# arnaucube/go-snark-study

Hardware: AMD Instinct MI355X
Metric: Groth16 constraints/sec (prove) at 2^20 R1CS (higher is better)
Workload: dtype u32 (9x29-bit Montgomery limbs of the 254-bit BN128 fields)

## Files before the change

go-snark-study_amd/csrc/msm.hip:

```cpp
#include "msm.h"
#include "hostcopy.h"

#include <algorithm>
#include <cmath>
#include <cstdlib>
#include <future>
#include <type_traits>

#include "msm_kernels.h"

namespace gs {

static_assert(sizeof(G1Xyzz) == PointIO<FqTag>::kXyzzWords * 4, "G1 XYZZ must be raw limbs");
static_assert(sizeof(G2Xyzz) == PointIO<Fq2Tag>::kXyzzWords * 4, "G2 XYZZ must be raw limbs");

int choose_window_bits(uint32_t n, int forced) {
  if (forced >= 8 && forced <= kMaxWindowBits) return forced;
  static const double per_bucket = dev_knob_f("GS_WINDOW_COST_BUCKET", 6.0, 0.0, 64.0);
  static const int auto_max = (int)dev_knob("GS_AUTO_MAX_C", 17, 8, kMaxWindowBits);
  int best = 8;
  double best_cost = 1e300;
  for (int c = 8; c <= std::min(kMaxWindowBits, std::max(8, auto_max)); ++c) {
    const int W = 254 / c + 1;
    const double cost = (double)n * W + per_bucket * (double)(1u << (c - 1));
    if (cost < best_cost) { best_cost = cost; best = c; }
  }
  return best;
}

int choose_window_bits_free(uint32_t n, int forced) {
  if (forced) return std::min(kMaxFreeWindowBits, std::max(kMinFreeWindowBits, forced));
  static const double per_bucket = dev_knob_f("GS_WINDOW_COST_BUCKET_FREE", 3.0, 0.0, 64.0);
  int best = kMinFreeWindowBits;
  double best_cost = 1e300;
  for (int c = kMinFreeWindowBits; c <= kMaxFreeWindowBits; ++c) {
    const int W = 254 / c + 1;
    const double cost = (double)W * ((double)n + per_bucket * (double)(1u << (c - 1)));
    if (cost < best_cost) { best_cost = cost; best = c; }
  }
  return best;
}

static void exclusive_scan(Ctx& c, PlanBuffers& pb, const uint32_t* in, uint32_t* out, uint32_t n) {
  const uint32_t ntiles = (n + kScanTile - 1) / kScanTile;
  pb.tiles.ensure((size_t)ntiles * 4);
  pb.total.ensure(4);
  hipLaunchKernelGGL(k_scan_tiles, dim3(ntiles), dim3(kScanBlock), 0, c.stream, in, out, pb.tiles.as<uint32_t>(), n);
  hipLaunchKernelGGL(k_scan_tile_sums, dim3(1), dim3(1024), 0, c.stream, pb.tiles.as<uint32_t>(), ntiles, pb.total.as<uint32_t>());
  hipLaunchKernelGGL(k_scan_add, dim3(ntiles), dim3(kScanBlock), 0, c.stream, out, pb.tiles.as<uint32_t>(), n);
}

struct MsmState {
  PlanBuffers plan_slots[3 * Ctx::kSlots];
  DevBuf upload_scratch;
  DevBuf upload_flag;
  bool lds_attr_set = false;
};
static MsmState& msm_state(Ctx& c) { return c.state<MsmState>(c.msm_state); }

static uint32_t choose_chunk(uint64_t entries, uint32_t nbuckets, const std::vector<LaunchShape>& users) {
  static const int forced = (int)dev_knob("GS_CHUNK", 0, 4, 1024, 4);
  if (forced >= 4 && forced % 4 == 0) return (uint32_t)forced;
  static const int forced_h = (int)dev_knob("GS_CHUNK_H", 0, 4, 1024, 4);
  if (forced_h && users.size() == 1 && users[0].njobs == 1 && !users[0].g2) return (uint32_t)forced_h;
  uint32_t chunk = entries >= (1ull << 27) ? 64u : entries >= (1ull << 23) ? 32u : 16u;
  while (chunk < 1024u && entries / std::max<uint32_t>(nbuckets, 1u) > 32ull * chunk) chunk *= 2;
  return chunk;
}

static uint32_t part_min_ranges() {
  static const uint32_t v = (uint32_t)dev_knob("GS_PART_MIN_R", 4, 2, 64);
  return v;
}
bool plan_partitions_first(int cbits) {
  if (cbits < 1) return false;
  return std::max<uint32_t>(1u, (1u << (cbits - 1)) >> kRangeLog) >= part_min_ranges();
}

uint32_t finite_mask_dev(Ctx& c, const uint32_t* g1_pts, const uint32_t* g2_pts, uint32_t n, uint32_t* mask_dev) {
  const size_t words = ((size_t)n + 31) / 32;
  GS_HIP(hipMemsetAsync(mask_dev, 0, std::max<size_t>(words, 1) * 4, c.stream));
  DevBuf cnt(4);
  GS_HIP(hipMemsetAsync(cnt.p, 0, 4, c.stream));
  if (n) hipLaunchKernelGGL(k_finite_mask, grid1(n), dim3(256), 0, c.stream, g1_pts, (uint32_t)PointIO<FqTag>::kAffineWords, g2_pts,
                            (uint32_t)PointIO<Fq2Tag>::kAffineWords, n, mask_dev, cnt.as<uint32_t>());
  GS_HIP(hipGetLastError());
  uint32_t host = 0;
  GS_HIP(hipMemcpyAsync(&host, cnt.p, 4, hipMemcpyDeviceToHost, c.stream));
  GS_HIP(hipStreamSynchronize(c.stream));
  return host;
}

void build_plan(Ctx& c, int slot, const uint32_t* scalars_dev, uint32_t n, MsmPlan& plan, const std::vector<LaunchShape>& users, int cbits,
                bool table_free, const uint32_t* term_index, uint32_t index_bias) {
  MsmState& ms = msm_state(c);
  PlanBuffers& pb = ms.plan_slots[slot % (3 * Ctx::kSlots)];
  plan.n = n;
  plan.table_free = table_free;
  plan.c = cbits ? cbits : (table_free ? choose_window_bits_free(n, c.window_bits) : choose_window_bits(n, c.window_bits));
  if (table_free && (plan.c < kMinFreeWindowBits || plan.c > kMaxFreeWindowBits))
    throw HipError{hipErrorInvalidValue, "table-free plan outside 9..16 window bits", __LINE__};
  plan.W = 254 / plan.c + 1;
  plan.B = 1u << (plan.c - 1);
  plan.nbuckets = table_free ? (uint32_t)plan.W * plan.B : plan.B;
  plan.chunk = choose_chunk((uint64_t)n * plan.W, plan.nbuckets, users);
  plan.maxchunks = (uint32_t)(((size_t)n * plan.W + plan.chunk - 1) / plan.chunk) + 1;
  const size_t ncount = (size_t)plan.nbuckets + 1;
  PlanParams pp{};
  pp.n = n; pp.c = plan.c; pp.W = plan.W; pp.B = plan.B;
  pp.R = std::max<uint32_t>(1u, plan.B >> kRangeLog);
  pp.tf = table_free ? 1u : 0u;
  {
    const uint32_t want = std::max<uint32_t>(1u, 256u / (plan.W * pp.R));
    const uint32_t by_size = std::max<uint32_t>(1u, (n + 16383u) / 16384u);
    const uint32_t by_mem = std::max<uint32_t>(1u, (uint32_t)((64ull << 20) / ((uint64_t)plan.B * plan.W * 4)));
    pp.S = std::max<uint32_t>(1u, std::min(std::min<uint32_t>(16u, std::max<uint32_t>(want, 1u)), std::min(by_size, by_mem)));
    if (pp.R == 1 && !table_free) pp.S = std::max<uint32_t>(1u, std::min<uint32_t>(16u, by_size));
  }
  pp.slice = (n + pp.S - 1) / pp.S;
  pp.stride = (n + 63u) & ~63u;
  const bool wide = plan_partitions_first(plan.c);
  if (wide && term_index) throw HipError{hipErrorInvalidValue, "plans over a term list cannot be sorted partition-first (plan_partitions_first)", __LINE__};
  const uint32_t nparts = (uint32_t)plan.W * pp.R;
  if (wide && nparts > kMaxParts) throw HipError{hipErrorInvalidValue, "too many (window, range) partitions", __LINE__};
  if (!wide) pb.digits.ensure((size_t)std::max<uint32_t>(pp.stride, 64u) * plan.W * sizeof(digit_t));
  else {
    pb.recs.ensure(std::max<size_t>((size_t)n * plan.W, 1) * 8);
    pb.parts.ensure((size_t)(3 * kMaxParts + 4) * 4);
  }
  pb.hist.ensure((size_t)plan.B * plan.W * pp.S * 4);
  pb.totals.ensure(ncount * 4);
  pb.offsets.ensure(ncount * 4);
  pb.entries.ensure(((size_t)plan.maxchunks + 1) * plan.chunk * 4);
  pb.chunk_bucket.ensure((size_t)plan.maxchunks * 4);
  pb.heavy_list.ensure((size_t)plan.nbuckets * 4);
  pb.counters.ensure(16);
  const size_t lds = (size_t)std::min<uint32_t>(plan.B, kRangeBuckets) * 4;
  static const int sort_block = (int)dev_knob("GS_SORT_BLOCK", kSortBlock, 64, kSortBlock, 64);
  if (!ms.lds_attr_set) {
    GS_HIP(hipFuncSetAttribute(reinterpret_cast<const void*>(k_hist), hipFuncAttributeMaxDynamicSharedMemorySize, 128 * 1024));
    GS_HIP(hipFuncSetAttribute(reinterpret_cast<const void*>(k_scatter), hipFuncAttributeMaxDynamicSharedMemorySize, 128 * 1024));
    GS_HIP(hipFuncSetAttribute(reinterpret_cast<const void*>(k_hist_part), hipFuncAttributeMaxDynamicSharedMemorySize, 128 * 1024));
    GS_HIP(hipFuncSetAttribute(reinterpret_cast<const void*>(k_scatter_part), hipFuncAttributeMaxDynamicSharedMemorySize, 128 * 1024));
    ms.lds_attr_set = true;
  }
  GS_HIP(hipMemsetAsync(pb.totals.as<uint32_t>() + plan.nbuckets, 0, 4, c.stream));
  GS_HIP(hipMemsetAsync(pb.counters.p, 0, 16, c.stream));
  uint32_t* part_count = pb.parts.as<uint32_t>();
  uint32_t* part_base = part_count ? part_count + kMaxParts : nullptr;
  uint32_t* part_cursor = part_count ? part_base + kMaxParts + 4 : nullptr;
  if (n > 0 && wide) {
    GS_HIP(hipMemsetAsync(part_count, 0, (size_t)nparts * 4, c.stream));
    hipLaunchKernelGGL(k_part_count, grid1(n, kPartBlock), dim3(kPartBlock), 0, c.stream, scalars_dev, pp, part_count);
    hipLaunchKernelGGL(k_part_scan, dim3(1), dim3(64), 0, c.stream, part_count, nparts, part_base, part_cursor);
    hipLaunchKernelGGL(k_part_scatter, grid1(n, kPartBlock * kPartPerThread), dim3(kPartBlock), 0, c.stream, scalars_dev, pp, part_base, part_cursor,
                       pb.recs.as<uint2>());
    hipLaunchKernelGGL(k_hist_part, dim3(8 * pp.S * ((nparts + 7) / 8)), dim3(sort_block), lds, c.stream, pb.recs.as<uint2>(), part_base, pp, pb.hist.as<uint32_t>());
    hipLaunchKernelGGL(k_colscan, grid1(plan.B), dim3(256), 0, c.stream, pb.hist.as<uint32_t>(), pp, pb.totals.as<uint32_t>());
  } else if (n > 0) {
    hipLaunchKernelGGL(k_digits, grid1(n), dim3(256), 0, c.stream, scalars_dev, pp, pb.digits.as<digit_t>(), term_index, index_bias);
    hipLaunchKernelGGL(k_hist, dim3(plan.W, pp.S, pp.R), dim3(sort_block), lds, c.stream, pb.digits.as<digit_t>(), pp, pb.hist.as<uint32_t>());
    if (table_free) hipLaunchKernelGGL(k_colscan_windows, grid1(plan.nbuckets), dim3(256), 0, c.stream, pb.hist.as<uint32_t>(), pp, pb.totals.as<uint32_t>());
    else hipLaunchKernelGGL(k_colscan, grid1(plan.B), dim3(256), 0, c.stream, pb.hist.as<uint32_t>(), pp, pb.totals.as<uint32_t>());
  } else {
    GS_HIP(hipMemsetAsync(pb.totals.p, 0, ncount * 4, c.stream));
  }
  exclusive_scan(c, pb, pb.totals.as<uint32_t>(), pb.offsets.as<uint32_t>(), (uint32_t)ncount);
  if (n > 0) {
    if (wide) hipLaunchKernelGGL(k_scatter_part, dim3(8 * pp.S * ((nparts + 7) / 8)), dim3(sort_block), lds, c.stream, pb.recs.as<uint2>(), part_base, pp,
                                 pb.hist.as<uint32_t>(), pb.offsets.as<uint32_t>(), pb.entries.as<uint32_t>());
    else hipLaunchKernelGGL(k_scatter, dim3(plan.W, pp.S, pp.R), dim3(sort_block), lds, c.stream, pb.digits.as<digit_t>(), pp, pb.hist.as<uint32_t>(),
                            pb.offsets.as<uint32_t>(), pb.entries.as<uint32_t>(), term_index, index_bias);
    hipLaunchKernelGGL(k_chunk_map, grid1(plan.nbuckets), dim3(256), 0, c.stream, pb.offsets.as<uint32_t>(), plan.nbuckets, plan.chunk,
                       pb.chunk_bucket.as<uint32_t>(), pb.heavy_list.as<uint32_t>(), pb.counters.as<uint32_t>());
  }
  GS_HIP(hipGetLastError());
  plan.offsets = pb.offsets.as<uint32_t>();
  plan.entries = pb.entries.as<uint32_t>();
  plan.chunk_bucket = pb.chunk_bucket.as<uint32_t>();
  plan.heavy_list = pb.heavy_list.as<uint32_t>();
  plan.heavy_count = pb.counters.as<uint32_t>();
}

template <class T>
static void msm_enqueue(Ctx& c, const MsmPlan& plan, const std::vector<MsmBase>& bases, int ws_base, int slot, MsmPending& p,
                        hipStream_t tail_stream) {
  const int njobs = (int)bases.size();
  p = MsmPending{};
  p.njobs = njobs; p.slot = slot; p.n = plan.n; p.g2 = PointIO<T>::kAffineWords == 32;
  p.c = plan.c; p.W = plan.W;
  if (njobs == 0 || plan.n == 0) { p.njobs = plan.n == 0 ? -njobs : 0; return; }
  if (njobs > kMaxJobs) throw HipError{hipErrorInvalidValue, "too many MSM jobs", __LINE__};
  constexpr size_t pw = PointIO<T>::kXyzzWords;
  constexpr size_t aw = PointIO<T>::kAffineWords;
  static const uint32_t fold_env = (uint32_t)dev_knob("GS_FOLD_MAX", 0, 1, 256);
  const uint32_t fold_max = fold_env ? fold_env : (plan.n >= (1u << 19) ? 32u : 16u);
  static const uint32_t l_min = (uint32_t)dev_knob("GS_REDUCE_L", 4, 1, 32, 1, true);
  int L = (int)std::max<uint32_t>(1u, std::min<uint32_t>(l_min, plan.B / kReduceBlock));
  while (L < 32 && plan.B / ((uint32_t)kReduceBlock * (uint32_t)L) > fold_max) L *= 2;
  uint32_t nblk = (plan.B + kReduceBlock * L - 1) / (kReduceBlock * L);
  if (plan.table_free) {
    L = (int)std::max<uint32_t>(1u, std::min<uint32_t>(16u, plan.B / kReduceBlock));
    p.nblk_window = plan.B / ((uint32_t)kReduceBlock * (uint32_t)L);
    nblk = p.nblk_window * (uint32_t)plan.W;
    p.table_free = true;
  }
  p.L = L; p.nblk = nblk;
  p.folded = !plan.table_free && nblk > fold_max;
  if (p.folded && nblk > (uint32_t)kReduceBlock) throw HipError{hipErrorInvalidValue, "too many reduce workgroups for one fold", __LINE__};
  const size_t pair_bytes = (size_t)njobs * nblk * 2 * pw * 4, final_bytes = (size_t)njobs * pw * 4, stats_bytes = 16;
  const size_t out_bytes = (p.folded ? final_bytes : pair_bytes + final_bytes) + stats_bytes;
  if (out_bytes > Ctx::kPinnedBytes) throw HipError{hipErrorInvalidValue, "MSM result staging too small", __LINE__};
  p.stats_off = out_bytes - stats_bytes;
  AccJobs jobs{};
  DevBuf& outb = c.ws_out[ws_base % Ctx::kWsSets];
  outb.ensure(pair_bytes + final_bytes + stats_bytes);
  uint32_t* finals = outb.as<uint32_t>() + pair_bytes / 4;
  uint32_t* stats = finals + final_bytes / 4;
  for (int j = 0; j < njobs; ++j) {
    const BaseTable* t = bases[j].table;
    const uint32_t* points = nullptr;
    uint32_t row_stride = 0;
    if (plan.table_free) {
      if (!bases[j].points || bases[j].off + plan.n > bases[j].npoints)
        throw HipError{hipErrorInvalidValue, "MSM base array does not cover the plan", __LINE__};
      points = bases[j].points + bases[j].off * aw;
    } else {
      if (!t || t->c != plan.c || !t->rows.p || bases[j].off + plan.n > t->n)
        throw HipError{hipErrorInvalidValue, "MSM base table does not match the plan", __LINE__};
      points = t->rows.as<uint32_t>() + bases[j].off * aw;
      row_stride = (uint32_t)t->n;
    }
    DevBuf& bk = c.ws_buckets[(ws_base + j) % Ctx::kWsSets];
    DevBuf& mg = c.ws_chunks[(ws_base + j) % Ctx::kWsSets];
    DevBuf& pt = c.ws_partials[(ws_base + j) % Ctx::kWsSets];
    bk.ensure((size_t)plan.nbuckets * pw * 4);
    mg.ensure((size_t)plan.nbuckets * pw * 4);
    pt.ensure((size_t)plan.maxchunks * 2 * pw * 4);
    jobs.j[j] = AccJob{points, row_stride, bk.as<uint32_t>(), pt.as<uint32_t>(),
                       pt.as<uint32_t>() + (size_t)plan.maxchunks * pw, mg.as<uint32_t>(),
                       outb.as<uint32_t>() + (size_t)j * nblk * 2 * pw, finals + (size_t)j * pw};
  }
  p.tacc = std::make_shared<PhaseTimer>(c.stream);
  p.tker = std::make_shared<PhaseTimer>(c.stream);
  hipLaunchKernelGGL(k_bucket_accumulate<T>, dim3((plan.maxchunks + kAccBlock - 1) / kAccBlock, njobs), dim3(kAccBlock), 0, c.stream,
                     jobs, plan.offsets, plan.entries, plan.chunk_bucket, plan.nbuckets, plan.chunk);
  p.tker->stop();
  p.tacc->stop();
  hipStream_t ts = tail_stream ? tail_stream : c.stream;
  if (ts != c.stream) {
    hipEvent_t ev;
    GS_HIP(hipEventCreateWithFlags(&ev, hipEventDisableTiming));
    GS_HIP(hipEventRecord(ev, c.stream));
    GS_HIP(hipStreamWaitEvent(ts, ev, 0));
    GS_HIP(hipEventDestroy(ev));
  }
  p.tred = std::make_shared<PhaseTimer>(ts);
  static const long alone_below_log2 = dev_knob("GS_TAIL_ALONE_LOG2", 19, 0, 32);
  const bool alone = plan.n < (1ull << alone_below_log2);
  auto launch_tails = [&](auto alone_tag) {
    constexpr bool kAlone = decltype(alone_tag)::value;
    hipLaunchKernelGGL((k_heavy_combine<T, kAlone>), dim3(64, njobs), dim3(kHeavyBlock), 0, ts,
                       jobs, plan.offsets, plan.heavy_list, plan.heavy_count, plan.chunk);
    hipLaunchKernelGGL((k_heavy_finish<T, kAlone>), dim3(16, njobs), dim3(kHeavyBlock), 0, ts,
                       jobs, plan.offsets, plan.heavy_list, plan.heavy_count, plan.chunk);
    hipLaunchKernelGGL((k_bucket_combine<T, kAlone>), dim3((plan.nbuckets + 255) / 256, njobs), dim3(256), 0, ts, jobs, plan.offsets, plan.nbuckets,
                       plan.chunk, plan.heavy_count, stats);
    hipLaunchKernelGGL((k_block_reduce<T, kAlone>), dim3(nblk, njobs), dim3(kReduceBlock), 0, ts, jobs, plan.nbuckets, L);
    if (p.folded) {
      int log2_span = 0;
      while ((1u << log2_span) < (uint32_t)kReduceBlock * (uint32_t)L) ++log2_span;
      hipLaunchKernelGGL((k_pair_reduce<T, kAlone>), dim3(1, njobs), dim3(kReduceBlock), 0, ts, jobs, nblk, log2_span);
    }
  };
  if (alone) launch_tails(std::true_type{}); else launch_tails(std::false_type{});
  GS_HIP(hipGetLastError());
  GS_HIP(hipMemcpyAsync(c.pinned[slot], p.folded ? (const void*)finals : outb.p, out_bytes, hipMemcpyDeviceToHost, ts));
  p.pinned_slot = c.pinned[slot];
  p.tred->stop();
}

template <class T>
static Xyzz<T> sum_pairs(const Xyzz<T>* pr, uint32_t nblk, int L) {
  Xyzz<T> run = xyzz_inf<T>(), tot = xyzz_inf<T>(), sumA = xyzz_inf<T>();
  for (uint32_t blk = nblk; blk-- > 0;) {
    xyzz_add(sumA, pr[2 * blk]);
    if (blk >= 1) { xyzz_add(run, pr[2 * blk + 1]); xyzz_add(tot, run); }
  }
  for (uint32_t s2 = (uint32_t)kReduceBlock * (uint32_t)L; s2 > 1; s2 >>= 1) xyzz_dbl(tot);
  xyzz_add(sumA, tot);
  return sumA;
}

void msm_book_timing(Ctx& c, const MsmPending& p) {
  if (p.njobs <= 0) return;
  std::lock_guard<std::mutex> lk(c.timing_mu);
  c.timing.accumulate_ms += p.tacc->ms();
  const uint64_t terms = (uint64_t)p.n * p.njobs;
  c.timing.window_bits = (uint32_t)p.c;
  c.timing.reduce_ms += p.tred->ms();
  const uint32_t* st = p.pinned_slot ? reinterpret_cast<const uint32_t*>(static_cast<const char*>(p.pinned_slot) + p.stats_off) : nullptr;
  const uint64_t adds = st ? (uint64_t)st[0] * p.njobs : terms * p.W;
  if (!p.g2) { c.timing.acc_g1_ms += p.tker->ms(); c.timing.acc_g1_launches += 1; c.timing.acc_g1_terms += terms; c.timing.acc_g1_adds += adds; }
  else { c.timing.acc_g2_ms += p.tker->ms(); c.timing.acc_g2_launches += 1; c.timing.acc_g2_terms += terms; c.timing.acc_g2_adds += adds; }
  c.timing.plan_digits += terms * p.W;
  c.timing.plan_entries += adds;
  if (st) c.timing.heavy_buckets += st[1];
}

template <class T>
static Xyzz<T> sum_pairs_windows(const Xyzz<T>* pr, const MsmPending& p) {
  Xyzz<T> acc = xyzz_inf<T>();
  for (int w = p.W; w-- > 0;) {
    for (int k = 0; k < p.c; ++k) xyzz_dbl(acc);
    xyzz_add(acc, sum_pairs<T>(pr + (size_t)w * p.nblk_window * 2, p.nblk_window, p.L));
  }
  return acc;
}

template <class T>
static void msm_finish(Ctx& c, const MsmPending& p, std::vector<Xyzz<T>>& out) {
  if (p.njobs <= 0) { out.assign(-p.njobs, xyzz_inf<T>()); return; }
  out.assign(p.njobs, xyzz_inf<T>());
  const Xyzz<T>* pairs = static_cast<const Xyzz<T>*>(c.pinned[p.slot]);
  if (p.folded) {
// ... 187 lines not shown
```

go-snark-study_amd/csrc/msm_kernels.h:

```cpp
#pragma once
#include <hip/hip_runtime.h>
#include <stdint.h>

#include "ec.h"
#include "point_io.h"
#include "zkey_convert.h"

namespace gs {

struct PlanParams {
  uint32_t n;
  int c;
  int W;
  uint32_t B;
  uint32_t S;
  uint32_t slice;
  uint32_t stride;
  uint32_t R;
  uint32_t tf;
};
constexpr uint32_t kRangeLog = 15;
constexpr uint32_t kRangeBuckets = 1u << kRangeLog;

GS_HD int32_t next_digit(const uint32_t (&k)[8], const PlanParams& pp, int w, uint32_t& carry) {
  uint32_t raw = scalar_bits(k, w * pp.c, pp.c) + carry;
  if (raw > pp.B) { carry = 1; return (int32_t)raw - (int32_t)(2u * pp.B); }
  carry = 0;
  return (int32_t)raw;
}

using digit_t = uint32_t;
__global__ void __launch_bounds__(256) k_digits(const uint32_t* __restrict__ scalars, PlanParams pp, digit_t* __restrict__ digits,
                                                 const uint32_t* __restrict__ term_index, uint32_t index_bias) {
  wave_priority<GS_PRIO_PLAN>();
  const uint32_t i = blockIdx.x * blockDim.x + threadIdx.x;
  if (i >= pp.n) return;
  const uint32_t src = term_index ? term_index[i] - index_bias : i;
  uint32_t k[8];
  const uint4* s4 = reinterpret_cast<const uint4*>(scalars + (size_t)src * 8);
  uint4 lo = s4[0], hi = s4[1];
  k[0] = lo.x; k[1] = lo.y; k[2] = lo.z; k[3] = lo.w; k[4] = hi.x; k[5] = hi.y; k[6] = hi.z; k[7] = hi.w;
  scalar_canon(k);
  uint32_t carry = 0;
  for (int w = 0; w < pp.W; ++w) {
    const int32_t d = next_digit(k, pp, w, carry);
    digits[(size_t)w * pp.stride + i] = (digit_t)(d + (int32_t)pp.B - 1);
  }
}

__global__ void __launch_bounds__(256) k_finite_mask(const uint32_t* __restrict__ a, uint32_t wa, const uint32_t* __restrict__ b, uint32_t wb, uint32_t n,
                                                      uint32_t* __restrict__ mask, uint32_t* __restrict__ count) {
  const uint32_t i = blockIdx.x * blockDim.x + threadIdx.x;
  bool finite = false;
  if (i < n) {
    uint32_t acc = 0;
    if (a) for (uint32_t k = 0; k < wa; ++k) acc |= a[(size_t)i * wa + k];
    if (b) for (uint32_t k = 0; k < wb; ++k) acc |= b[(size_t)i * wb + k];
    finite = acc != 0;
  }
  if (finite) { atomicOr(&mask[i >> 5], 1u << (i & 31u)); atomicAdd(count, 1u); }
}

constexpr int kSortBlock = 1024;

__global__ void __launch_bounds__(kSortBlock) k_hist(const digit_t* __restrict__ digits, PlanParams pp, uint32_t* __restrict__ hist) {
  wave_priority<GS_PRIO_PLAN>();
  extern __shared__ uint32_t sh[];
  const uint32_t w = blockIdx.x, s = blockIdx.y, r = blockIdx.z;
  const uint32_t nb = min(pp.B, kRangeBuckets), base = r << kRangeLog;
  for (uint32_t b = threadIdx.x; b < nb; b += blockDim.x) sh[b] = 0;
  __syncthreads();
  const uint32_t lo = s * pp.slice, hi = min(pp.n, lo + pp.slice);
  const digit_t* row = digits + (size_t)w * pp.stride;
  const int32_t zero = (int32_t)pp.B - 1;
  for (uint32_t i = lo + threadIdx.x; i < hi; i += blockDim.x) {
    const int32_t d = (int32_t)row[i] - zero;
    if (d != 0) {
      const uint32_t b = (uint32_t)(d < 0 ? -d : d) - 1u;
      if ((b >> kRangeLog) == r) atomicAdd(&sh[b - base], 1u);
    }
  }
  __syncthreads();
  uint32_t* out = hist + ((size_t)w * pp.S + s) * pp.B + base;
  for (uint32_t b = threadIdx.x; b < nb; b += blockDim.x) out[b] = sh[b];
}

__global__ void __launch_bounds__(256) k_colscan(uint32_t* __restrict__ hist, PlanParams pp, uint32_t* __restrict__ totals) {
  wave_priority<GS_PRIO_PLAN>();
  const uint32_t b = blockIdx.x * blockDim.x + threadIdx.x;
  if (b >= pp.B) return;
  uint32_t* col = hist + b;
  const uint32_t nq = (uint32_t)pp.W * pp.S;
  uint32_t run = 0;
  for (uint32_t q = 0; q < nq; ++q) { const uint32_t t = col[(size_t)q * pp.B]; col[(size_t)q * pp.B] = run; run += t; }
  totals[b] = run;
}

__global__ void __launch_bounds__(256) k_colscan_windows(uint32_t* __restrict__ hist, PlanParams pp, uint32_t* __restrict__ totals) {
  wave_priority<GS_PRIO_PLAN>();
  const uint32_t i = blockIdx.x * blockDim.x + threadIdx.x;
  if (i >= (uint32_t)pp.W * pp.B) return;
  const uint32_t w = i / pp.B, b = i % pp.B;
  uint32_t* col = hist + (size_t)w * pp.S * pp.B + b;
  uint32_t run = 0;
  for (uint32_t q = 0; q < pp.S; ++q) { const uint32_t t = col[(size_t)q * pp.B]; col[(size_t)q * pp.B] = run; run += t; }
  totals[i] = run;
}

__global__ void __launch_bounds__(kSortBlock) k_scatter(const digit_t* __restrict__ digits, PlanParams pp, const uint32_t* __restrict__ hist,
                                                         const uint32_t* __restrict__ offsets, uint32_t* __restrict__ entries,
                                                         const uint32_t* __restrict__ term_index, uint32_t index_bias) {
  wave_priority<GS_PRIO_PLAN>();
  extern __shared__ uint32_t sh[];
  const uint32_t w = blockIdx.x, s = blockIdx.y, r = blockIdx.z;
  const uint32_t nb = min(pp.B, kRangeBuckets), base = r << kRangeLog;
  const uint32_t* pre = hist + ((size_t)w * pp.S + s) * pp.B + base;
  const uint32_t* off = offsets + (pp.tf ? (size_t)w * pp.B : (size_t)0);
  for (uint32_t b = threadIdx.x; b < nb; b += blockDim.x) sh[b] = off[base + b] + pre[b];
  __syncthreads();
  const uint32_t lo = s * pp.slice, hi = min(pp.n, lo + pp.slice);
  const digit_t* row = digits + (size_t)w * pp.stride;
  const int32_t zero = (int32_t)pp.B - 1;
  for (uint32_t i = lo + threadIdx.x; i < hi; i += blockDim.x) {
    const int32_t d = (int32_t)row[i] - zero;
    if (d != 0) {
      const uint32_t b = (uint32_t)(d < 0 ? -d : d) - 1u;
      if ((b >> kRangeLog) == r) {
        const uint32_t pos = atomicAdd(&sh[b - base], 1u);
        const uint32_t id = term_index ? term_index[i] - index_bias : i;
        entries[pos] = id | (w << kWindowShift) | (d < 0 ? kSignBit : 0u);
      }
    }
  }
}

constexpr int kPartBlock = 256;
constexpr int kPartPerThread = 4;
constexpr uint32_t kMaxParts = 512;

GS_HD void load_scalar_canon(const uint32_t* __restrict__ scalars, uint32_t i, uint32_t (&k)[8]) {
  const uint4* s4 = reinterpret_cast<const uint4*>(scalars + (size_t)i * 8);
  const uint4 lo = s4[0], hi = s4[1];
  k[0] = lo.x; k[1] = lo.y; k[2] = lo.z; k[3] = lo.w; k[4] = hi.x; k[5] = hi.y; k[6] = hi.z; k[7] = hi.w;
  scalar_canon(k);
}

__global__ void __launch_bounds__(kPartBlock) k_part_count(const uint32_t* __restrict__ scalars, PlanParams pp, uint32_t* __restrict__ part_count) {
  wave_priority<GS_PRIO_PLAN>();
  __shared__ uint32_t cnt[kMaxParts];
  const uint32_t nparts = (uint32_t)pp.W * pp.R;
  for (uint32_t t = threadIdx.x; t < nparts; t += kPartBlock) cnt[t] = 0;
  __syncthreads();
  const uint32_t i = blockIdx.x * kPartBlock + threadIdx.x;
  if (i < pp.n) {
    uint32_t k[8];
    load_scalar_canon(scalars, i, k);
    uint32_t carry = 0;
    for (int w = 0; w < pp.W; ++w) {
      const int32_t d = next_digit(k, pp, w, carry);
      if (d != 0) atomicAdd(&cnt[(uint32_t)w * pp.R + (((uint32_t)(d < 0 ? -d : d) - 1u) >> kRangeLog)], 1u);
    }
  }
  __syncthreads();
  for (uint32_t t = threadIdx.x; t < nparts; t += kPartBlock) if (cnt[t]) atomicAdd(&part_count[t], cnt[t]);
}

__global__ void __launch_bounds__(64) k_part_scan(uint32_t* __restrict__ part_count, uint32_t nparts, uint32_t* __restrict__ part_base,
                                                    uint32_t* __restrict__ part_cursor) {
  wave_priority<GS_PRIO_PLAN>();
  if (blockIdx.x != 0 || threadIdx.x != 0) return;
  uint32_t run = 0;
  for (uint32_t t = 0; t < nparts; ++t) { part_base[t] = run; run += part_count[t]; part_cursor[t] = 0; part_count[t] = 0; }
  part_base[nparts] = run;
}

__global__ void __launch_bounds__(kPartBlock) k_part_scatter(const uint32_t* __restrict__ scalars, PlanParams pp, const uint32_t* __restrict__ part_base,
                                                              uint32_t* __restrict__ part_cursor, uint2* __restrict__ recs) {
  wave_priority<GS_PRIO_PLAN>();
  __shared__ uint32_t cnt[kMaxParts];
  const uint32_t nparts = (uint32_t)pp.W * pp.R;
  for (uint32_t t = threadIdx.x; t < nparts; t += kPartBlock) cnt[t] = 0;
  __syncthreads();
  const uint32_t first = blockIdx.x * (kPartBlock * kPartPerThread);
  for (int j = 0; j < kPartPerThread; ++j) {
    const uint32_t i = first + j * kPartBlock + threadIdx.x;
    if (i >= pp.n) break;
    uint32_t k[8];
    load_scalar_canon(scalars, i, k);
    uint32_t carry = 0;
    for (int w = 0; w < pp.W; ++w) {
      const int32_t d = next_digit(k, pp, w, carry);
      if (d != 0) atomicAdd(&cnt[(uint32_t)w * pp.R + (((uint32_t)(d < 0 ? -d : d) - 1u) >> kRangeLog)], 1u);
    }
  }
  __syncthreads();
  for (uint32_t t = threadIdx.x; t < nparts; t += kPartBlock) {
    const uint32_t mine = cnt[t];
    cnt[t] = part_base[t] + (mine ? atomicAdd(&part_cursor[t], mine) : 0u);
  }
  __syncthreads();
  for (int j = 0; j < kPartPerThread; ++j) {
    const uint32_t i = first + j * kPartBlock + threadIdx.x;
    if (i >= pp.n) break;
    uint32_t k[8];
    load_scalar_canon(scalars, i, k);
    uint32_t carry = 0;
    for (int w = 0; w < pp.W; ++w) {
      const int32_t d = next_digit(k, pp, w, carry);
      if (d != 0) {
        const uint32_t b = (uint32_t)(d < 0 ? -d : d) - 1u;
        const uint32_t pos = atomicAdd(&cnt[(uint32_t)w * pp.R + (b >> kRangeLog)], 1u);
        recs[pos] = make_uint2(i | (d < 0 ? kSignBit : 0u), b);
      }
    }
  }
}

GS_HD bool part_of_block(uint32_t id, const PlanParams& pp, uint32_t& w, uint32_t& r, uint32_t& s) {
  const uint32_t xcd = id & 7u, j = id >> 3;
  const uint32_t p = xcd + 8u * (j / pp.S);
  s = j % pp.S;
  w = p / pp.R; r = p % pp.R;
  return p < (uint32_t)pp.W * pp.R;
}

GS_HD void part_slice(const uint32_t* __restrict__ part_base, const PlanParams& pp, uint32_t w, uint32_t r, uint32_t s, uint32_t& lo, uint32_t& hi) {
  const uint32_t p0 = part_base[w * pp.R + r], p1 = part_base[w * pp.R + r + 1];
  const uint32_t len = p1 - p0, per = (len + pp.S - 1) / pp.S;
  lo = min(p1, p0 + s * per);
  hi = min(p1, lo + per);
}

__global__ void __launch_bounds__(kSortBlock) k_hist_part(const uint2* __restrict__ recs, const uint32_t* __restrict__ part_base, PlanParams pp,
                                                           uint32_t* __restrict__ hist) {
  wave_priority<GS_PRIO_PLAN>();
  extern __shared__ uint32_t sh[];
  uint32_t w, r, s;
  if (!part_of_block(blockIdx.x, pp, w, r, s)) return;
  const uint32_t base = r << kRangeLog;
  for (uint32_t b = threadIdx.x; b < kRangeBuckets; b += blockDim.x) sh[b] = 0;
  __syncthreads();
  uint32_t lo, hi;
  part_slice(part_base, pp, w, r, s, lo, hi);
  for (uint32_t e = lo + threadIdx.x; e < hi; e += blockDim.x) atomicAdd(&sh[recs[e].y - base], 1u);
  __syncthreads();
  uint32_t* out = hist + ((size_t)w * pp.S + s) * pp.B + base;
  for (uint32_t b = threadIdx.x; b < kRangeBuckets; b += blockDim.x) out[b] = sh[b];
}

__global__ void __launch_bounds__(kSortBlock) k_scatter_part(const uint2* __restrict__ recs, const uint32_t* __restrict__ part_base, PlanParams pp,
                                                              const uint32_t* __restrict__ hist, const uint32_t* __restrict__ offsets,
                                                              uint32_t* __restrict__ entries) {
  wave_priority<GS_PRIO_PLAN>();
  extern __shared__ uint32_t sh[];
  uint32_t w, r, s;
  if (!part_of_block(blockIdx.x, pp, w, r, s)) return;
  const uint32_t base = r << kRangeLog;
  const uint32_t* pre = hist + ((size_t)w * pp.S + s) * pp.B + base;
  for (uint32_t b = threadIdx.x; b < kRangeBuckets; b += blockDim.x) sh[b] = offsets[base + b] + pre[b];
  __syncthreads();
  uint32_t lo, hi;
  part_slice(part_base, pp, w, r, s, lo, hi);
  for (uint32_t e = lo + threadIdx.x; e < hi; e += blockDim.x) {
    const uint2 rec = recs[e];
    entries[atomicAdd(&sh[rec.y - base], 1u)] = rec.x | (w << kWindowShift);
  }
}

constexpr int kScanBlock = 256;
constexpr int kScanPerThread = 8;
constexpr int kScanTile = kScanBlock * kScanPerThread;

__global__ void __launch_bounds__(kScanBlock) k_scan_tiles(const uint32_t* __restrict__ in, uint32_t* __restrict__ out,
                                                            uint32_t* __restrict__ tile_sums, uint32_t n) {
  wave_priority<GS_PRIO_PLAN>();
  __shared__ uint32_t sh[kScanBlock];
  const uint32_t base = blockIdx.x * kScanTile + threadIdx.x * kScanPerThread;
  uint32_t v[kScanPerThread], sum = 0;
#pragma unroll
  for (int j = 0; j < kScanPerThread; ++j) { v[j] = (base + j < n) ? in[base + j] : 0u; sum += v[j]; }
  sh[threadIdx.x] = sum;
  __syncthreads();
  for (int off = 1; off < kScanBlock; off <<= 1) {
    uint32_t t = (threadIdx.x >= (uint32_t)off) ? sh[threadIdx.x - off] : 0u;
    __syncthreads();
// ... 481 lines not shown
```

Measured before the change: 123.6 million.

## Pack MSM sort digits as narrow magnitudes with ballot skip/sign bitplanes

The digit array for the non-partitioned sort path changes layout. Each entry becomes a 16-bit magnitude when the window width is at most 17 bits, and the skip and sign flags move into per-wave 64-bit ballot bitplanes. The histogram and scatter kernels now read eight digits per vector load together with byte masks, use a 1D grid that groups windows by XCD, and work on slices aligned to 64. Column scans are batched eight at a time. The aim is to cut memory traffic and load instruction count in the plan phase, at the cost of more complex indexing and two kernel instantiations.

```diff
diff --git a/go-snark-study_amd/csrc/msm.hip b/go-snark-study_amd/csrc/msm.hip
--- a/go-snark-study_amd/csrc/msm.hip
+++ b/go-snark-study_amd/csrc/msm.hip
@@ -117,13 +117,15 @@
     pp.S = std::max<uint32_t>(1u, std::min(std::min<uint32_t>(16u, std::max<uint32_t>(want, 1u)), std::min(by_size, by_mem)));
     if (pp.R == 1 && !table_free) pp.S = std::max<uint32_t>(1u, std::min<uint32_t>(16u, by_size));
   }
-  pp.slice = (n + pp.S - 1) / pp.S;
+  pp.slice = sort_slice_terms(n, pp.S);
   pp.stride = (n + 63u) & ~63u;
   const bool wide = plan_partitions_first(plan.c);
   if (wide && term_index) throw HipError{hipErrorInvalidValue, "plans over a term list cannot be sorted partition-first (plan_partitions_first)", __LINE__};
   const uint32_t nparts = (uint32_t)plan.W * pp.R;
   if (wide && nparts > kMaxParts) throw HipError{hipErrorInvalidValue, "too many (window, range) partitions", __LINE__};
-  if (!wide) pb.digits.ensure((size_t)std::max<uint32_t>(pp.stride, 64u) * plan.W * sizeof(digit_t));
+  const bool narrow_digits = plan.c <= kNarrowDigitBits;
+  const size_t mag_bytes = std::max<size_t>(digit_mag_bytes(pp), 64);
+  if (!wide) pb.digits.ensure(mag_bytes + std::max<size_t>(digit_plane_words(pp), 2) * 8);
   else {
     pb.recs.ensure(std::max<size_t>((size_t)n * plan.W, 1) * 8);
     pb.parts.ensure((size_t)(3 * kMaxParts + 4) * 4);
@@ -138,8 +140,10 @@
   const size_t lds = (size_t)std::min<uint32_t>(plan.B, kRangeBuckets) * 4;
   static const int sort_block = (int)dev_knob("GS_SORT_BLOCK", kSortBlock, 64, kSortBlock, 64);
   if (!ms.lds_attr_set) {
-    GS_HIP(hipFuncSetAttribute(reinterpret_cast<const void*>(k_hist), hipFuncAttributeMaxDynamicSharedMemorySize, 128 * 1024));
-    GS_HIP(hipFuncSetAttribute(reinterpret_cast<const void*>(k_scatter), hipFuncAttributeMaxDynamicSharedMemorySize, 128 * 1024));
+    GS_HIP(hipFuncSetAttribute(reinterpret_cast<const void*>(k_hist<uint16_t>), hipFuncAttributeMaxDynamicSharedMemorySize, 128 * 1024));
+    GS_HIP(hipFuncSetAttribute(reinterpret_cast<const void*>(k_hist<uint32_t>), hipFuncAttributeMaxDynamicSharedMemorySize, 128 * 1024));
+    GS_HIP(hipFuncSetAttribute(reinterpret_cast<const void*>(k_scatter<uint16_t>), hipFuncAttributeMaxDynamicSharedMemorySize, 128 * 1024));
+    GS_HIP(hipFuncSetAttribute(reinterpret_cast<const void*>(k_scatter<uint32_t>), hipFuncAttributeMaxDynamicSharedMemorySize, 128 * 1024));
     GS_HIP(hipFuncSetAttribute(reinterpret_cast<const void*>(k_hist_part), hipFuncAttributeMaxDynamicSharedMemorySize, 128 * 1024));
     GS_HIP(hipFuncSetAttribute(reinterpret_cast<const void*>(k_scatter_part), hipFuncAttributeMaxDynamicSharedMemorySize, 128 * 1024));
     ms.lds_attr_set = true;
@@ -149,6 +153,17 @@
   uint32_t* part_count = pb.parts.as<uint32_t>();
   uint32_t* part_base = part_count ? part_count + kMaxParts : nullptr;
   uint32_t* part_cursor = part_count ? part_base + kMaxParts + 4 : nullptr;
+  uint64_t* planes = wide ? nullptr : reinterpret_cast<uint64_t*>(static_cast<char*>(pb.digits.p) + mag_bytes);
+  auto launch_digits = [&](auto* mags) {
+    using D = std::remove_pointer_t<decltype(mags)>;
+    hipLaunchKernelGGL(k_digits<D>, grid1(pp.stride), dim3(256), 0, c.stream, scalars_dev, pp, mags, planes, term_index, index_bias);
+    hipLaunchKernelGGL(k_hist<D>, dim3(sort_grid(pp)), dim3(sort_block), lds, c.stream, mags, planes, pp, pb.hist.as<uint32_t>());
+  };
+  auto launch_scatter = [&](auto* mags) {
+    using D = std::remove_pointer_t<decltype(mags)>;
+    hipLaunchKernelGGL(k_scatter<D>, dim3(sort_grid(pp)), dim3(sort_block), lds, c.stream, mags, planes, pp, pb.hist.as<uint32_t>(),
+                       pb.offsets.as<uint32_t>(), pb.entries.as<uint32_t>(), term_index, index_bias);
+  };
   if (n > 0 && wide) {
     GS_HIP(hipMemsetAsync(part_count, 0, (size_t)nparts * 4, c.stream));
     hipLaunchKernelGGL(k_part_count, grid1(n, kPartBlock), dim3(kPartBlock), 0, c.stream, scalars_dev, pp, part_count);
@@ -158,8 +173,7 @@
     hipLaunchKernelGGL(k_hist_part, dim3(8 * pp.S * ((nparts + 7) / 8)), dim3(sort_block), lds, c.stream, pb.recs.as<uint2>(), part_base, pp, pb.hist.as<uint32_t>());
     hipLaunchKernelGGL(k_colscan, grid1(plan.B), dim3(256), 0, c.stream, pb.hist.as<uint32_t>(), pp, pb.totals.as<uint32_t>());
   } else if (n > 0) {
-    hipLaunchKernelGGL(k_digits, grid1(n), dim3(256), 0, c.stream, scalars_dev, pp, pb.digits.as<digit_t>(), term_index, index_bias);
-    hipLaunchKernelGGL(k_hist, dim3(plan.W, pp.S, pp.R), dim3(sort_block), lds, c.stream, pb.digits.as<digit_t>(), pp, pb.hist.as<uint32_t>());
+    if (narrow_digits) launch_digits(pb.digits.as<uint16_t>()); else launch_digits(pb.digits.as<uint32_t>());
     if (table_free) hipLaunchKernelGGL(k_colscan_windows, grid1(plan.nbuckets), dim3(256), 0, c.stream, pb.hist.as<uint32_t>(), pp, pb.totals.as<uint32_t>());
     else hipLaunchKernelGGL(k_colscan, grid1(plan.B), dim3(256), 0, c.stream, pb.hist.as<uint32_t>(), pp, pb.totals.as<uint32_t>());
   } else {
@@ -169,8 +183,8 @@
   if (n > 0) {
     if (wide) hipLaunchKernelGGL(k_scatter_part, dim3(8 * pp.S * ((nparts + 7) / 8)), dim3(sort_block), lds, c.stream, pb.recs.as<uint2>(), part_base, pp,
                                  pb.hist.as<uint32_t>(), pb.offsets.as<uint32_t>(), pb.entries.as<uint32_t>());
-    else hipLaunchKernelGGL(k_scatter, dim3(plan.W, pp.S, pp.R), dim3(sort_block), lds, c.stream, pb.digits.as<digit_t>(), pp, pb.hist.as<uint32_t>(),
-                            pb.offsets.as<uint32_t>(), pb.entries.as<uint32_t>(), term_index, index_bias);
+    else if (narrow_digits) launch_scatter(pb.digits.as<uint16_t>());
+    else launch_scatter(pb.digits.as<uint32_t>());
     hipLaunchKernelGGL(k_chunk_map, grid1(plan.nbuckets), dim3(256), 0, c.stream, pb.offsets.as<uint32_t>(), plan.nbuckets, plan.chunk,
                        pb.chunk_bucket.as<uint32_t>(), pb.heavy_list.as<uint32_t>(), pb.counters.as<uint32_t>());
   }
diff --git a/go-snark-study_amd/csrc/msm_kernels.h b/go-snark-study_amd/csrc/msm_kernels.h
--- a/go-snark-study_amd/csrc/msm_kernels.h
+++ b/go-snark-study_amd/csrc/msm_kernels.h
@@ -29,22 +29,48 @@
   return (int32_t)raw;
 }
 
-using digit_t = uint32_t;
-__global__ void __launch_bounds__(256) k_digits(const uint32_t* __restrict__ scalars, PlanParams pp, digit_t* __restrict__ digits,
+constexpr int kNarrowDigitBits = 17;
+struct DigitCode { uint32_t mag; bool neg, skip; };
+GS_HD DigitCode digit_encode(int32_t d) {
+  DigitCode e;
+  e.skip = d == 0;
+  e.neg = d < 0;
+  e.mag = e.skip ? 0u : (uint32_t)(d < 0 ? -d : d) - 1u;
+  return e;
+}
+GS_HD int32_t digit_decode(uint32_t mag, bool neg, bool skip) {
+  if (skip) return 0;
+  return neg ? -(int32_t)(mag + 1u) : (int32_t)(mag + 1u);
+}
+GS_HD size_t digit_mag_bytes(const PlanParams& pp) { return (size_t)pp.stride * pp.W * (pp.c <= kNarrowDigitBits ? 2 : 4); }
+GS_HD size_t digit_plane_words(const PlanParams& pp) { return (size_t)pp.W * 2 * (pp.stride >> 6); }
+template <class D> struct alignas(sizeof(D) * 8) Digit8 { D v[8]; };
+
+template <class D>
+__global__ void __launch_bounds__(256) k_digits(const uint32_t* __restrict__ scalars, PlanParams pp, D* __restrict__ mags, uint64_t* __restrict__ planes,
                                                  const uint32_t* __restrict__ term_index, uint32_t index_bias) {
   wave_priority<GS_PRIO_PLAN>();
   const uint32_t i = blockIdx.x * blockDim.x + threadIdx.x;
-  if (i >= pp.n) return;
-  const uint32_t src = term_index ? term_index[i] - index_bias : i;
-  uint32_t k[8];
-  const uint4* s4 = reinterpret_cast<const uint4*>(scalars + (size_t)src * 8);
-  uint4 lo = s4[0], hi = s4[1];
-  k[0] = lo.x; k[1] = lo.y; k[2] = lo.z; k[3] = lo.w; k[4] = hi.x; k[5] = hi.y; k[6] = hi.z; k[7] = hi.w;
-  scalar_canon(k);
+  if (i >= pp.stride) return;
+  uint32_t k[8] = {0, 0, 0, 0, 0, 0, 0, 0};
+  if (i < pp.n) {
+    const uint32_t src = term_index ? term_index[i] - index_bias : i;
+    const uint4* s4 = reinterpret_cast<const uint4*>(scalars + (size_t)src * 8);
+    uint4 lo = s4[0], hi = s4[1];
+    k[0] = lo.x; k[1] = lo.y; k[2] = lo.z; k[3] = lo.w; k[4] = hi.x; k[5] = hi.y; k[6] = hi.z; k[7] = hi.w;
+    scalar_canon(k);
+  }
+  const uint32_t words = pp.stride >> 6;
   uint32_t carry = 0;
   for (int w = 0; w < pp.W; ++w) {
-    const int32_t d = next_digit(k, pp, w, carry);
-    digits[(size_t)w * pp.stride + i] = (digit_t)(d + (int32_t)pp.B - 1);
+    const DigitCode e = digit_encode(next_digit(k, pp, w, carry));
+    mags[(size_t)w * pp.stride + i] = (D)e.mag;
+    const uint64_t skip = __ballot(e.skip), neg = __ballot(e.neg);
+    if ((threadIdx.x & 63u) == 0) {
+      uint64_t* p = planes + (size_t)w * 2 * words + (i >> 6);
+      p[0] = skip;
+      p[words] = neg;
+    }
   }
 }
 
@@ -63,37 +89,72 @@
 
 constexpr int kSortBlock = 1024;
 
-__global__ void __launch_bounds__(kSortBlock) k_hist(const digit_t* __restrict__ digits, PlanParams pp, uint32_t* __restrict__ hist) {
+GS_HD uint32_t sort_grid(const PlanParams& pp) { return 8u * pp.S * pp.R * (((uint32_t)pp.W + 7u) / 8u); }
+GS_HD bool sort_block_of(uint32_t id, const PlanParams& pp, uint32_t& w, uint32_t& s, uint32_t& r) {
+  const uint32_t xcd = id & 7u, j = id >> 3, per = pp.S * pp.R;
+  w = xcd + 8u * (j / per);
+  s = (j % per) / pp.R;
+  r = (j % per) % pp.R;
+  return w < (uint32_t)pp.W;
+}
+GS_HD uint32_t sort_slice_terms(uint32_t n, uint32_t S) { return ((n + S - 1u) / S + 63u) & ~63u; }
+GS_HD void sort_slice_groups(const PlanParams& pp, uint32_t s, uint32_t& lo, uint32_t& hi) {
+  const uint32_t first = min(s * pp.slice, pp.stride);
+  lo = first >> 3;
+  hi = min(first + pp.slice, pp.stride) >> 3;
+}
+
+template <class D>
+__global__ void __launch_bounds__(kSortBlock) k_hist(const D* __restrict__ mags, const uint64_t* __restrict__ planes, PlanParams pp,
+                                                      uint32_t* __restrict__ hist) {
   wave_priority<GS_PRIO_PLAN>();
   extern __shared__ uint32_t sh[];
-  const uint32_t w = blockIdx.x, s = blockIdx.y, r = blockIdx.z;
+  uint32_t w, s, r;
+  if (!sort_block_of(blockIdx.x, pp, w, s, r)) return;
   const uint32_t nb = min(pp.B, kRangeBuckets), base = r << kRangeLog;
   for (uint32_t b = threadIdx.x; b < nb; b += blockDim.x) sh[b] = 0;
   __syncthreads();
-  const uint32_t lo = s * pp.slice, hi = min(pp.n, lo + pp.slice);
-  const digit_t* row = digits + (size_t)w * pp.stride;
-  const int32_t zero = (int32_t)pp.B - 1;
-  for (uint32_t i = lo + threadIdx.x; i < hi; i += blockDim.x) {
-    const int32_t d = (int32_t)row[i] - zero;
-    if (d != 0) {
-      const uint32_t b = (uint32_t)(d < 0 ? -d : d) - 1u;
-      if ((b >> kRangeLog) == r) atomicAdd(&sh[b - base], 1u);
-    }
+  uint32_t lo, hi;
+  sort_slice_groups(pp, s, lo, hi);
+  const Digit8<D>* row = reinterpret_cast<const Digit8<D>*>(mags + (size_t)w * pp.stride);
+  const uint8_t* skip = reinterpret_cast<const uint8_t*>(planes + (size_t)w * 2 * (pp.stride >> 6));
+  auto count = [&](const Digit8<D>& d, uint32_t sk) {
+#pragma unroll
+    for (int j = 0; j < 8; ++j) {
+      const uint32_t b = d.v[j];
+      if (!((sk >> j) & 1u) && (b >> kRangeLog) == r) atomicAdd(&sh[b - base], 1u);
+    }
+  };
+  for (uint32_t g = lo + threadIdx.x; g < hi; g += 2 * blockDim.x) {
+    const uint32_t g2 = g + blockDim.x < hi ? g + blockDim.x : g;
+    const Digit8<D> d0 = row[g], d1 = row[g2];
+    const uint32_t s0 = skip[g], s1 = g2 != g ? skip[g2] : 0xffu;
+    count(d0, s0);
+    count(d1, s1);
   }
   __syncthreads();
   uint32_t* out = hist + ((size_t)w * pp.S + s) * pp.B + base;
   for (uint32_t b = threadIdx.x; b < nb; b += blockDim.x) out[b] = sh[b];
 }
 
+GS_HD uint32_t colscan_column(uint32_t* __restrict__ col, size_t pitch, uint32_t nq) {
+  constexpr uint32_t kBatch = 8;
+  uint32_t run = 0;
+  for (uint32_t q0 = 0; q0 < nq; q0 += kBatch) {
+    uint32_t t[kBatch];
+#pragma unroll
+    for (uint32_t j = 0; j < kBatch; ++j) t[j] = q0 + j < nq ? col[(size_t)(q0 + j) * pitch] : 0u;
+#pragma unroll
+    for (uint32_t j = 0; j < kBatch; ++j) if (q0 + j < nq) { col[(size_t)(q0 + j) * pitch] = run; run += t[j]; }
+  }
+  return run;
+}
+
 __global__ void __launch_bounds__(256) k_colscan(uint32_t* __restrict__ hist, PlanParams pp, uint32_t* __restrict__ totals) {
   wave_priority<GS_PRIO_PLAN>();
   const uint32_t b = blockIdx.x * blockDim.x + threadIdx.x;
   if (b >= pp.B) return;
-  uint32_t* col = hist + b;
-  const uint32_t nq = (uint32_t)pp.W * pp.S;
-  uint32_t run = 0;
-  for (uint32_t q = 0; q < nq; ++q) { const uint32_t t = col[(size_t)q * pp.B]; col[(size_t)q * pp.B] = run; run += t; }
-  totals[b] = run;
+  totals[b] = colscan_column(hist + b, pp.B, (uint32_t)pp.W * pp.S);
 }
 
 __global__ void __launch_bounds__(256) k_colscan_windows(uint32_t* __restrict__ hist, PlanParams pp, uint32_t* __restrict__ totals) {
@@ -101,36 +162,47 @@
   const uint32_t i = blockIdx.x * blockDim.x + threadIdx.x;
   if (i >= (uint32_t)pp.W * pp.B) return;
   const uint32_t w = i / pp.B, b = i % pp.B;
-  uint32_t* col = hist + (size_t)w * pp.S * pp.B + b;
-  uint32_t run = 0;
-  for (uint32_t q = 0; q < pp.S; ++q) { const uint32_t t = col[(size_t)q * pp.B]; col[(size_t)q * pp.B] = run; run += t; }
-  totals[i] = run;
-}
-
-__global__ void __launch_bounds__(kSortBlock) k_scatter(const digit_t* __restrict__ digits, PlanParams pp, const uint32_t* __restrict__ hist,
-                                                         const uint32_t* __restrict__ offsets, uint32_t* __restrict__ entries,
-                                                         const uint32_t* __restrict__ term_index, uint32_t index_bias) {
+  totals[i] = colscan_column(hist + (size_t)w * pp.S * pp.B + b, pp.B, pp.S);
+}
+
+template <class D>
+__global__ void __launch_bounds__(kSortBlock) k_scatter(const D* __restrict__ mags, const uint64_t* __restrict__ planes, PlanParams pp,
+                                                         const uint32_t* __restrict__ hist, const uint32_t* __restrict__ offsets,
+                                                         uint32_t* __restrict__ entries, const uint32_t* __restrict__ term_index, uint32_t index_bias) {
   wave_priority<GS_PRIO_PLAN>();
   extern __shared__ uint32_t sh[];
-  const uint32_t w = blockIdx.x, s = blockIdx.y, r = blockIdx.z;
+  uint32_t w, s, r;
+  if (!sort_block_of(blockIdx.x, pp, w, s, r)) return;
   const uint32_t nb = min(pp.B, kRangeBuckets), base = r << kRangeLog;
   const uint32_t* pre = hist + ((size_t)w * pp.S + s) * pp.B + base;
   const uint32_t* off = offsets + (pp.tf ? (size_t)w * pp.B : (size_t)0);
   for (uint32_t b = threadIdx.x; b < nb; b += blockDim.x) sh[b] = off[base + b] + pre[b];
   __syncthreads();
-  const uint32_t lo = s * pp.slice, hi = min(pp.n, lo + pp.slice);
-  const digit_t* row = digits + (size_t)w * pp.stride;
-  const int32_t zero = (int32_t)pp.B - 1;
-  for (uint32_t i = lo + threadIdx.x; i < hi; i += blockDim.x) {
-    const int32_t d = (int32_t)row[i] - zero;
-    if (d != 0) {
-      const uint32_t b = (uint32_t)(d < 0 ? -d : d) - 1u;
-      if ((b >> kRangeLog) == r) {
+  uint32_t lo, hi;
+  sort_slice_groups(pp, s, lo, hi);
+  const Digit8<D>* row = reinterpret_cast<const Digit8<D>*>(mags + (size_t)w * pp.stride);
+  const uint8_t* skip = reinterpret_cast<const uint8_t*>(planes + (size_t)w * 2 * (pp.stride >> 6));
+  const uint8_t* neg = skip + ((size_t)(pp.stride >> 6) << 3);
+  const uint32_t tag = w << kWindowShift;
+  auto place = [&](uint32_t g, const Digit8<D>& d, uint32_t sk, uint32_t ng) {
+#pragma unroll
+    for (int j = 0; j < 8; ++j) {
+      const uint32_t b = d.v[j];
+      if (!((sk >> j) & 1u) && (b >> kRangeLog) == r) {
         const uint32_t pos = atomicAdd(&sh[b - base], 1u);
+        const uint32_t i = g * 8u + (uint32_t)j;
         const uint32_t id = term_index ? term_index[i] - index_bias : i;
-        entries[pos] = id | (w << kWindowShift) | (d < 0 ? kSignBit : 0u);
+        entries[pos] = id | tag | (((ng >> j) & 1u) ? kSignBit : 0u);
       }
     }
+  };
+  for (uint32_t g = lo + threadIdx.x; g < hi; g += 2 * blockDim.x) {
+    const uint32_t g2 = g + blockDim.x < hi ? g + blockDim.x : g;
+    const Digit8<D> d0 = row[g], d1 = row[g2];
+    const uint32_t s0 = skip[g], s1 = g2 != g ? skip[g2] : 0xffu;
+    const uint32_t n0 = neg[g], n1 = neg[g2];
+    place(g, d0, s0, n0);
+    place(g2, d1, s1, n1);
   }
 }
 
```

Result: faster. 126.2 million (median of 6 runs) (+2.1%).
